# bottledspace/refraction-raytracing-dxr

Hardware: AMD Instinct MI355X
Metric: Mrays/s (primary+refracted) at 1920x1080, monkey.obj (higher is better)
Workload: dtype f32

## Files before the change

### refraction_raytracing_dxr_amd/csrc/rr_capi.cpp

```cpp
#include "../../include/rrdxr.h"

#include <hip/hip_runtime.h>

#include <algorithm>
#include <cmath>
#include <cstdio>
#include <cstdlib>
#include <cstring>
#include <new>
#include <string>
#include <vector>

#include "rr_launch.h"

using namespace rr;

static_assert(sizeof(rr_vertex) == 32, "Vertex stride (Mesh.cpp:45)");
static_assert(sizeof(rr_instance_desc) == 64, "D3D12_RAYTRACING_INSTANCE_DESC");
static_assert(sizeof(rr_scene_constants) == 80, "SceneConstants");
static_assert(sizeof(rr_ray) == sizeof(rr_ray_dev) && sizeof(rr_hit) == sizeof(rr_hit_dev), "ray/hit ABI");
static_assert(offsetof(rr_ray, instance_mask) == 36 && offsetof(rr_ray_dev, instance_mask) == 36, "rr_ray.instance_mask");

#include <dlfcn.h>
struct rr_nccl_unique_id { char internal[128]; };
// ... 127 lines not shown
    size_t    park_bytes[MAX_LANES + 1] = {};
    char       last_kernel_name[96] = "";
    uint32_t   last_kernel = 0;
    uint32_t* d_tickets = nullptr;

    int  dbg_kernel = 0;
    int  dbg_stack = 0;
    int  dbg_ticket_blocks = 0;
    bool dbg_group_trace = true;
    bool dbg_async_set = false;
    uint32_t dbg_async[2] = { 2, 2 };
    bool dbg_tile_order = true;
    int  dbg_stream_waves = 6;
    bool dbg_tlas32 = false;
    int  dbg_shape = 0;
    std::string dbg_diag;

    hipEvent_t ev_begin = nullptr, ev_end = nullptr;
    std::vector<hipEvent_t> kev;
    uint32_t kev_used = 0;

    StreamDev strm[MAX_LANES + 1] = {};
    size_t    strm_cap[MAX_LANES + 1] = {};
    size_t    strm_pixels[MAX_LANES + 1] = {};
    size_t    strm_budget = 0;
    struct KernelChoice {
        int choice = 0;
        uint32_t seen = 0;
        unsigned long long key = 0;
        double share = 0.0;
// ... 13 lines not shown
                if (x.stamp < lru->stamp) lru = &x;
            }
            *lru = KernelChoice();
            lru->valid = true; lru->key = key; lru->stamp = clock;
            return lru;
        }
        const KernelChoice* peek(unsigned long long key) const
        {
            for (const KernelChoice& x : e) if (x.valid && x.key == key) return &x;
            return nullptr;
        }
    };
    static unsigned long long choice_key(uint32_t width, uint32_t height, const rr_dispatch_params& p, uint32_t depth)
    {
        return ((unsigned long long)width << 48) ^ ((unsigned long long)height << 32) ^ ((unsigned long long)(uint32_t)p.max_refract << 8) ^
               ((unsigned long long)(uint32_t)p.max_reflect << 4) ^ (depth <= 2 ? depth : depth < 8 ? 3u : depth < 24 ? 4u : depth < 48 ? 5u : 6u);
    }
    ChoiceClass ch_tlas, ch_many, ch_few;
    hipEvent_t ch_ev[4] = {};

    rr_ray_dev* d_rays = nullptr;
    rr_hit_dev* d_hits = nullptr;
    uint32_t ray_cap = 0;
};

namespace {

int fail(rr_context* ctx, int code, const char* what, hipError_t e = hipSuccess)
{
    if (ctx) {
        ctx->err = what;
// ... 162 lines not shown
        hipMalloc(&ctx->d_cnt, sizeof(CounterBlock)) != hipSuccess ||
        hipMalloc(&ctx->d_tickets, (rr_context::MAX_LANES + 1) * LDS_TICKET_WORDS * sizeof(uint32_t)) != hipSuccess) {
        if (ctx->own_stream) (void)hipStreamDestroy(ctx->own_stream);
        dfree(ctx->d_cnt);
        delete ctx;
        return RR_ERR_DEVICE;
    }
    ctx->stream = ctx->own_stream;
    (void)hipMemsetAsync(ctx->d_cnt, 0, sizeof(CounterBlock), ctx->stream);
    (void)hipMemsetAsync(ctx->d_tickets, 0, (rr_context::MAX_LANES + 1) * LDS_TICKET_WORDS * sizeof(uint32_t), ctx->stream);
    if (const char* e = getenv("RR_DEBUG_KERNEL"))
        ctx->dbg_kernel = !strcmp(e, "fused") ? 1 : !strcmp(e, "lds") ? 4 : !strcmp(e, "paths") ? 5 : !strcmp(e, "stream") ? 10 : 0;
    if (const char* e = getenv("RR_DEBUG_STACK")) ctx->dbg_stack = atoi(e);
    if (const char* e = getenv("RR_DEBUG_TICKET")) ctx->dbg_ticket_blocks = atoi(e);
    if (const char* e = getenv("RR_DEBUG_SHAPE")) ctx->dbg_shape = atoi(e);
    if (const char* e = getenv("RR_DEBUG_TLAS32")) ctx->dbg_tlas32 = atoi(e) != 0;
    if (const char* e = getenv("RR_DEBUG_TILE_ORDER")) ctx->dbg_tile_order = atoi(e) != 0;
    if (const char* e = getenv("RR_DEBUG_ASYNC")) { unsigned l = 2, sh = 2; if (sscanf(e, "%u,%u", &l, &sh) == 2 && l >= 1 && sh >= 1) { ctx->dbg_async[0] = l; ctx->dbg_async[1] = sh; ctx->dbg_async_set = true; } }
    if (const char* e = getenv("RR_DEBUG_DIAG")) ctx->dbg_diag = e;
    if (const char* e = getenv("RR_DEBUG_GROUP_TRACE")) ctx->dbg_group_trace = atoi(e) != 0;
    *out = ctx;
    return RR_OK;
}

int rr_destroy(rr_context* ctx)
{
    if (!ctx) return RR_ERR_INVALID_ARGUMENT;
    (void)hipSetDevice(ctx->device);
    (void)hipStreamSynchronize(ctx->stream);
    for (uint32_t l = 0; l < rr_context::MAX_LANES; ++l) {
// ... 543 lines not shown
constexpr size_t STREAM_BUDGET_MAX = (size_t)48 << 30, STREAM_BUDGET_MIN = (size_t)1 << 30;
constexpr uint32_t STREAM_BLK = 1024;

size_t stream_budget(rr_context* ctx)
{
    if (ctx->strm_budget == 0) {
        size_t free_b = 0, total_b = 0;
        size_t b = STREAM_BUDGET_MAX;
        if (hipMemGetInfo(&free_b, &total_b) == hipSuccess) b = std::min(b, free_b / 6u);
        if (const char* e = getenv("RR_DEBUG_STREAM_BUDGET_GB")) { const long g = atol(e); if (g > 0 && g <= 200) b = (size_t)g << 30; }
        ctx->strm_budget = std::max(b, STREAM_BUDGET_MIN);
    }
    return ctx->strm_budget;
}

inline bool lds_default_depth(uint32_t depth) { return depth >= 24u; }

bool scene_fits_lds(const rr_context* ctx)
{
    if (!ctx->single_identity || ctx->dbg_stack != 0 || ctx->inst_host.empty()) return false;
    const MeshRes& m0 = ctx->meshes[(size_t)ctx->inst_host[0].blas];
    const uint32_t node_bytes = (m0.n_tris > 1 ? m0.n_tris - 1 : 1) * (uint32_t)sizeof(QNode);
    return m0.n_tris < 32768u && lds_kernel_shape(node_bytes, scene_stack_need(ctx) + 1, nullptr, ctx->dbg_shape) >= 0;
}

uint32_t stream_slot(const rr_context* ctx)
{
    for (uint32_t l = 0; l < rr_context::MAX_LANES; ++l) if (ctx->lane_stream[l] && ctx->stream == ctx->lane_stream[l]) return l;
    return rr_context::MAX_LANES;
}

struct StreamPlan { uint32_t fc, n_wg; size_t cap, pixels; };

size_t stream_rect_wb(const DispatchDev& a, uint32_t frames)
{
    const size_t all = (size_t)a.blocks_per_frame * frames * 4u;
    if (!a.mesh_part && a.rt_w == 0u) return all;
    const size_t tiles = a.mesh_part ? (size_t)a.n_mesh_local : (size_t)a.rt_w * a.rt_h;
// ... 178 lines not shown
        RR_HIP(hipMemsetAsync(d_diag, 0, diag_waves * 64, ctx->stream));
        a.diag = d_diag;
    }

    const bool stats = (p.flags & RR_DISPATCH_COLLECT_STATS) != 0;
    const uint32_t need = scene_stack_need(ctx);
    const bool keep = keep_counters || (p.flags & RR_DISPATCH_KEEP_COUNTERS) != 0;
    const uint32_t filled = mesh ? n_mesh_local : local;
    if (compact && filled < max_local)
        for (uint32_t f = 0; f < depth; ++f)
            RR_HIP(hipMemsetAsync(reinterpret_cast<uint8_t*>(a.out_rgba8 + f * stride) + (size_t)filled * TILE * TILE * (rgb8 ? 3 : 4), 0,
                                  (size_t)(max_local - filled) * TILE * TILE * (rgb8 ? 3 : 4), ctx->stream));
    int stack_sel = need <= 19 ? 19 : need <= 22 ? 22 : need <= 26 ? 26 : need <= 31 ? 31 : need <= 39 ? 39 : 64;
    if (ctx->dbg_stack >= (int)need) stack_sel = ctx->dbg_stack;
    const MeshRes* m0 = ctx->single_identity ? &ctx->meshes[(size_t)ctx->inst_host[0].blas] : nullptr;
    const uint32_t node_bytes = m0 ? (m0->n_tris > 1 ? m0->n_tris - 1 : 1) * (uint32_t)sizeof(QNode) : 0;
    const double rect_share = (double)(a.hx1 - a.hx0) * (double)(a.hy1 - a.hy0) / ((double)width * (double)height);
    const bool lds_fits = scene_fits_lds(ctx) && (uint64_t)a.n_tiles * depth * depth < 0x40000000ull;
    const bool have_rect = a.hx1 > a.hx0 && a.hy1 > a.hy0;
    uint32_t pool_nodes = 0;
    if (!ctx->single_identity) {
        pool_nodes = ctx->n_insts > 1 ? ctx->n_insts - 1 : 1;
        std::vector<char> seen(ctx->meshes.size(), 0);
        for (uint32_t i = 0; i < ctx->n_insts; ++i) {
            const size_t mi = (size_t)ctx->inst_host[i].blas;
            if (!seen[mi]) { seen[mi] = 1; pool_nodes += ctx->meshes[mi].n_tris > 1 ? ctx->meshes[mi].n_tris - 1 : 1; }
        }
    }
    const bool refill_stack16 = ctx->single_identity ? (m0 && m0->n_tris < 32768u && need > 19)
                                                     : (pool_nodes < 32768u && ctx->n_pool_tris + ctx->n_insts < 32768u);
    const bool stream_ok = !ctx->single_identity && p.max_reflect <= 2 && p.max_refract <= (int)STREAM_MAX_GEN - 2 && refill_stack16 && need <= 39 &&
// ... 25 lines not shown
    auto launch_lds = [&](bool st) -> int {
        LdsDispatch q;
        memset(&q, 0, sizeof q);
        const uint32_t slot = lds_slot();
        q.tickets = ctx->d_tickets + (size_t)slot * LDS_TICKET_WORDS;
        q.park_slots = p.max_reflect <= 2 ? 2u : 8u;
        if (int r = ensure_lds_park(slot)) return r;
        q.park = ctx->d_park[slot];
        uint32_t rect[4];
        mesh_screen_rect(m0->bounds, ((ctx->dbg_ticket_blocks & 3) == 1 || (p.flags & RR_DISPATCH_DEBUG_NO_CULL)) ? nullptr : h_cams, depth, width, height, rect);
        const int tk = ctx->dbg_ticket_blocks & 3;
        if (tk == 2) rect[2] = rect[0];
        q.n_queues = (ctx->dbg_ticket_blocks & 64) ? 64u : (ctx->dbg_ticket_blocks & 128) ? LDS_QUEUES : 8u;
        q.home_xcc = (ctx->dbg_ticket_blocks & 16) ? 0u : 1u;
        q.rx0 = rect[0]; q.ry0 = rect[1]; q.rx1 = rect[2]; q.ry1 = rect[3];
        q.node_bytes = node_bytes;
        q.stack_entries = need + 1;
        RR_HIP(launch_render_lds(sc, a, q, ctx->n_cus, st, ctx->stream, ctx->dbg_shape));
        return RR_OK;
    };
    auto launch_paths = [&](bool st) -> int { RR_HIP(launch_render_paths(sc, a, (int)need, st, ctx->stream)); return RR_OK; };
    auto launch_stream = [&](bool st) -> int { return render_stream(ctx, sc, a, depth, (int)need, st, rgb8); };

    enum { K_FUSED = 0, K_LDS = 1, K_PATHS = 2, K_STREAM = 7 };
    int kernel = K_FUSED;
    rr_context::ChoiceClass* cls = nullptr;
    int cand_a = K_FUSED, cand_b = K_FUSED;
    if (ctx->dbg_kernel == 10) { if (stream_ok) kernel = K_STREAM; }
    else if (ctx->dbg_kernel == 5) { if (paths_ok) kernel = K_PATHS; }
    else if (ctx->dbg_kernel == 4) { if (lds_fits && !mesh && !compact) kernel = K_LDS; }
    else if (ctx->dbg_kernel == 0 && !a.diag) {
        if (stream_ok) { cls = &ctx->ch_tlas; cand_b = K_STREAM; }
        else if (paths_ok) { cls = &ctx->ch_few; cand_b = K_PATHS; }
// ... 805 lines not shown
```

### refraction_raytracing_dxr_amd/csrc/rr_device.h

```cpp
#pragma once
#include <hip/hip_runtime.h>
#include "rr_types.h"

namespace rr {

struct f3 { float x, y, z; };

__device__ __forceinline__ f3 mk3(float x, float y, float z) { f3 r; r.x = x; r.y = y; r.z = z; return r; }
__device__ __forceinline__ f3 sub3(f3 a, f3 b) { return mk3(a.x - b.x, a.y - b.y, a.z - b.z); }
__device__ __forceinline__ f3 neg3(f3 a) { return mk3(-a.x, -a.y, -a.z); }
__device__ __forceinline__ f3 scale3(f3 a, float s) { return mk3(a.x * s, a.y * s, a.z * s); }
__device__ __forceinline__ float dot3(f3 a, f3 b) { return fmaf(a.z, b.z, fmaf(a.y, b.y, a.x * b.x)); }
__device__ __forceinline__ f3 cross3(f3 a, f3 b)
{
    return mk3(fmaf(a.y, b.z, -(a.z * b.y)), fmaf(a.z, b.x, -(a.x * b.z)), fmaf(a.x, b.y, -(a.y * b.x)));
}
__device__ __forceinline__ f3 normalize3(f3 a)
{
    float inv = 1.0f / sqrtf(dot3(a, a));
    return scale3(a, inv);
}

__device__ __forceinline__ float rr_atan2f(float y, float x)
{
// ... 85 lines not shown
    BoxRay r;
    box_axis(O.x, D.x, eps_w, g.org[0], g.cell[0], r.inv.x, r.kn.x, r.kf.x, r.sx);
    box_axis(O.y, D.y, eps_w, g.org[1], g.cell[1], r.inv.y, r.kn.y, r.kf.y, r.sy);
    box_axis(O.z, D.z, eps_w, g.org[2], g.cell[2], r.inv.z, r.kn.z, r.kf.z, r.sz);
    return r;
}

struct NodeQ { uint4 a, b; };
__device__ __forceinline__ NodeQ load_node(const QNode* __restrict__ nodes, int node)
{
    const uint4* q = reinterpret_cast<const uint4*>(reinterpret_cast<const char*>(nodes) + (uint32_t)node);
    NodeQ n;
    n.a = q[0]; n.b = q[1];
    return n;
}
struct GlobalNodes {
    __device__ __forceinline__ NodeQ load(const QNode* __restrict__ nodes, int node) const { return load_node(nodes, node); }
};
struct LdsNodes {
    const char* base;
    __device__ __forceinline__ NodeQ load(const QNode* __restrict__, int node) const
    {
        const uint4* q = reinterpret_cast<const uint4*>(base + (uint32_t)node);
        NodeQ n;
        n.a = q[0]; n.b = q[1];
        return n;
    }
};


constexpr int TRAV_DONE = (int)0x80000000;

typedef float v2f __attribute__((ext_vector_type(2)));
__device__ __forceinline__ v2f splat2(float x) { v2f r = { x, x }; return r; }
__device__ __forceinline__ v2f mk2(float x, float y) { v2f r = { x, y }; return r; }

__device__ __forceinline__ float vmax3(float a, float b, float c) { float r; asm("v_max3_f32 %0, %1, %2, %3" : "=v"(r) : "v"(a), "v"(b), "v"(c)); return r; }
__device__ __forceinline__ float vmin3(float a, float b, float c) { float r; asm("v_min3_f32 %0, %1, %2, %3" : "=v"(r) : "v"(a), "v"(b), "v"(c)); return r; }
__device__ __forceinline__ float vmax2(float a, float b) { float r; asm("v_max_f32 %0, %1, %2" : "=v"(r) : "v"(a), "v"(b)); return r; }
__device__ __forceinline__ float vmin2(float a, float b) { float r; asm("v_min_f32 %0, %1, %2" : "=v"(r) : "v"(a), "v"(b)); return r; }

typedef _Float16 h2v __attribute__((ext_vector_type(2)));
// ... 5 lines not shown
    const uint32_t lox = n.a.x, loy = n.a.y, loz = n.a.z, hix = n.a.w, hiy = n.b.x, hiz = n.b.y;
    const v2f nx = RR_PLANE2(r.sx ? hix : lox, r.inv.x, r.kn.x);
    const v2f ny = RR_PLANE2(r.sy ? hiy : loy, r.inv.y, r.kn.y);
    const v2f nz = RR_PLANE2(r.sz ? hiz : loz, r.inv.z, r.kn.z);
    const v2f fx = RR_PLANE2(r.sx ? lox : hix, r.inv.x, r.kf.x);
    const v2f fy = RR_PLANE2(r.sy ? loy : hiy, r.inv.y, r.kf.y);
    const v2f fz = RR_PLANE2(r.sz ? loz : hiz, r.inv.z, r.kf.z);
    tn0 = vmax2(vmax3(nx.x, ny.x, nz.x), tmin);
    tn1 = vmax2(vmax3(nx.y, ny.y, nz.y), tmin);
    const float tf0 = vmin2(vmin3(fx.x, fy.x, fz.x), tmax);
    const float tf1 = vmin2(vmin3(fx.y, fy.y, fz.y), tmax);
    h0 = tn0 <= tf0;
    h1 = tn1 <= tf1;
}

constexpr int STACK_STRIDE = 64;
template <class E> struct StackCodec;
template <> struct StackCodec<uint32_t> {
    static __device__ __forceinline__ uint32_t enc(int ref) { return (uint32_t)ref; }
    static __device__ __forceinline__ int dec(uint32_t v) { return (int)v; }
};
template <> struct StackCodec<uint16_t> {
    static __device__ __forceinline__ uint16_t enc(int ref) { const int n = ref >> 5; return (uint16_t)(n < ref ? n : ref); }
    static __device__ __forceinline__ int dec(uint16_t v) { const int s = (int)(int16_t)v, n = s << 5; return n > s ? n : s; }
};

template <class E>
__device__ __forceinline__ int node_step(const BoxRay& br, const NodeQ& n, float tmin, float tmax, E*& top, const E* floor)
{
    bool h0, h1;
    float tn0, tn1;
    box2_hit(br, n, tmin, tmax, h0, h1, tn0, tn1);
    const int c0 = (int)n.b.z, c1 = (int)n.b.w;
    const bool both = h0 && h1, swap = tn1 < tn0;
    const int nearc = (h0 && !(h1 && swap)) ? c0 : c1;
    int next = (h0 || h1) ? nearc : TRAV_DONE;
    if (both) { *top = StackCodec<E>::enc(swap ? c0 : c1); top += STACK_STRIDE; }
    if (!(h0 || h1) && top > floor) { top -= STACK_STRIDE; next = StackCodec<E>::dec(*top); }
    return next;
}

struct Diag { uint32_t* trips; uint32_t stride = 4; };
__device__ __forceinline__ void diag_trip(const Diag& d, int which = 0)
{
    if (d.trips) { const unsigned long long m = __ballot(1); if ((int)(threadIdx.x & 63u) == __ffsll((long long)m) - 1) d.trips[which * d.stride] += 1u; }
}


__device__ __forceinline__ void tri_test(const TriRec* __restrict__ tris, uint32_t leaf, f3 O, f3 D, float tmin,
                                         uint32_t cull, uint32_t inst, HitRec& best)
{
    const float4* q = reinterpret_cast<const float4*>(tris + leaf);
    float4 a = q[0], b = q[1], c = q[2];
    f3 v0 = mk3(a.x, a.y, a.z), e1 = mk3(b.x, b.y, b.z), e2 = mk3(c.x, c.y, c.z);
    uint32_t prim = __float_as_uint(a.w);
// ... 37 lines not shown
__device__ __forceinline__ bool leaf_phase_due(int n_in)
{
    const int quarter = n_in >> 2;
    const int thr = quarter > 2 ? quarter : 2;
    return __popcll(__ballot(1)) + thr <= n_in;
}

template <bool STATS, class E, class NS = GlobalNodes, bool ANY = false>
__device__ __forceinline__ void walk_blas(const QNode* __restrict__ nodes, const TriRec* __restrict__ tris, int root, const BoxRay& br,
                                          f3 O, f3 D, float tmin, uint32_t cull, uint32_t inst, HitRec& best, E* stk,
                                          TravCounters& cnt, const Diag dg = Diag{ nullptr }, const NS ns = NS{},
                                          bool any_lane = false)
{
    E* top = stk;
    int node = root;
    for (;;) {
        const int n_in = __popcll(__ballot(node >= 0));
        while (node >= 0) {
            if (leaf_phase_due(n_in)) break;
            diag_trip(dg);
            const NodeQ q = ns.load(nodes, node);
            if (STATS) { cnt.nodes++; if (first_active_lane()) cnt.node_trips++; }
            node = node_step(br, q, tmin, best.t, top, stk);
#ifdef RR_EXP_EXTRA_VALU
            { float dv = br.inv.x;
#pragma unroll
              for (int k = 0; k < RR_EXP_EXTRA_VALU; ++k) asm volatile("v_add_f32 %0, %0, %0" : "+v"(dv));
              asm volatile("" :: "v"(dv)); }
#endif
        }
        if (node < 0 && node != TRAV_DONE) {
            diag_trip(dg, 1);
            if (STATS) { cnt.tris++; if (first_active_lane()) cnt.leaf_trips++; }
            tri_test(tris, (uint32_t)~node, O, D, tmin, cull, inst, best);
            if (ANY && any_lane && best.hit) { top = stk; node = TRAV_DONE; }
            else if (top > stk) { top -= STACK_STRIDE; node = StackCodec<E>::dec(*top); } else node = TRAV_DONE;
        }
        if (__ballot(node != TRAV_DONE) == 0ull) break;
    }
}

template <bool STATS, class E, class NS = GlobalNodes>
__device__ __forceinline__ void trace_blas(const BlasDev& bl, f3 O, f3 D, float tmin, uint32_t cull, uint32_t inst,
                                           HitRec& best, E* stk, TravCounters& cnt, const Diag dg = Diag{ nullptr },
                                           const NS ns = NS{})
{
    const BoxRay br = box_ray(O, D, bl.scale, bl.grid);
    walk_blas<STATS, E, NS>(bl.nodes, bl.tris, 0, br, O, D, tmin, cull, inst, best, stk, cnt, dg, ns);
    if (best.hit) hit_attributes(bl.tris, O, D, best);
}

// ... 244 lines not shown
```

### refraction_raytracing_dxr_amd/csrc/rr_launch.h

```cpp
#pragma once
#include <hip/hip_runtime.h>
#include "rr_types.h"

namespace rr {

struct alignas(16) rr_ray_dev { float origin[3]; float tmin; float dir[3]; float tmax; uint32_t flags; uint32_t instance_mask; uint32_t pad[2]; };
struct rr_hit_dev { float t, u, v; uint32_t prim, inst, hit; };
static_assert(sizeof(rr_ray_dev) == 48 && sizeof(rr_hit_dev) == 24, "ABI layout");

hipError_t launch_render_fused(const SceneDev& sc, const DispatchDev& a, int stack, int pend, bool stats, hipStream_t s,
                               bool stack16 = false);
int lds_kernel_shape(uint32_t node_bytes, uint32_t stack_entries, size_t* lds_bytes, int min_shape = 0);
hipError_t launch_render_lds(const SceneDev& sc, const DispatchDev& a, LdsDispatch q, int n_cus, bool stats, hipStream_t s, int min_shape = 0);
hipError_t launch_render_paths(const SceneDev& sc, const DispatchDev& a, int stack, bool stats, hipStream_t s);
hipError_t launch_assemble_frames_mesh_rgb8(const uint8_t* gathered, const uint8_t* bg, uint32_t* frames, uint32_t W, uint32_t H, const MeshPartDev& mp,
                                            size_t rank_stride_b, size_t frame_stride_b, size_t bg_stride_b, size_t out_stride, uint32_t n_frames, hipStream_t s);
hipError_t launch_render_stream(const SceneDev& sc, const DispatchDev& a, const StreamDev& s, int stack, uint32_t n_wg, bool stats, hipStream_t st, int waves = 6);
const char* last_stream_kernel_name();
const char* last_render_kernel_name();
hipError_t launch_trace_rays(const SceneDev& sc, const rr_ray_dev* rays, uint32_t n, rr_hit_dev* hits, uint32_t* err,
                             int stack, hipStream_t s);
hipError_t launch_query_rays(const SceneDev& sc, const rr_ray_dev* rays, uint32_t n, rr_hit_dev* hits, uint32_t inst0_mask, int stack,
                             hipStream_t s);
hipError_t launch_screen_tables(float* out, uint32_t W, uint32_t H, hipStream_t s);
hipError_t launch_env_lookup(const SceneDev& sc, const float* dirs, uint32_t n, float* rgb, hipStream_t s);
hipError_t launch_assemble_tiles(const uint32_t* gathered, uint32_t* frame, uint32_t W, uint32_t H, uint32_t tiles_x,
                                 uint32_t n_tiles, uint32_t world, uint32_t max_tiles, hipStream_t s);
hipError_t launch_assemble_frames(const uint32_t* gathered, uint32_t* frames, uint32_t W, uint32_t H, uint32_t tiles_x,
// ... 42 lines not shown
```

### refraction_raytracing_dxr_amd/csrc/rr_render.hip

```cpp
#include <hip/hip_runtime.h>
#include <cstdlib>
#include <cstring>
#include "rr_render_common.h"

namespace rr {

template <int STACK, int PEND, bool STATS, bool TLAS, bool DIAG = false, class E = uint32_t, int WPS = 0>
__global__ __launch_bounds__(256, WPS ? WPS : TLAS ? RR_TLAS_WAVES_PER_SIMD(STACK) : sizeof(E) == 2 ? 8 : RR_FUSED_WAVES_PER_SIMD(STACK)) void k_render_fused(SceneDev sc, DispatchDev a)
{
    __shared__ uint32_t diag_trips[12];
    const unsigned long long diag_t0 = DIAG ? __builtin_amdgcn_s_memtime() : 0ull;
    const unsigned long long diag_rt0 = DIAG ? __builtin_amdgcn_s_memrealtime() : 0ull;
    if (DIAG && threadIdx.x < 12) diag_trips[threadIdx.x] = 0;
    if (DIAG) __syncthreads();
    extern __shared__ __attribute__((aligned(16))) uint32_t lds[];
    const uint32_t wave = __builtin_amdgcn_readfirstlane(threadIdx.x >> 6), lane = threadIdx.x & 63u;
    E* stk = reinterpret_cast<E*>(lds) + wave * (STACK * 64) + lane;

    const BlockPos bp = wave_block_pos(a, blockIdx.x * 4u + wave);
    const uint32_t lx = compact1by1(lane), ly = compact1by1(lane >> 1);
    const uint32_t x = bp.x0 + lx, y = bp.y0 + ly;
    const bool valid = bp.tile_ok && x < a.W && y < a.H;
    const CamDev& cb = a.cams[bp.frame];

// ... 208 lines not shown
    return p;
}

__device__ __forceinline__ BlockPos lds_rect_block(const DispatchDev& a, const LdsDispatch& q, uint32_t u, uint32_t j)
{
    BlockPos p;
    const uint32_t strip = a.n_frames == 1u ? u : __umulhi(u, q.div_frames), per_row = q.rect_bw >> 2;
    p.frame = u - strip * a.n_frames;
    const uint32_t row = per_row == 1u ? strip : __umulhi(strip, q.div_per_row), col = strip - row * per_row;
    p.tile_local = 0u; p.tile_ok = true; p.bg = false;
    p.px0 = 0u; p.py0 = 0u;
    p.x0 = q.rx0 + col * 32u + j * 8u; p.y0 = q.ry0 + row * 8u;
    return p;
}

template <int NW, int WGS, bool STATS, bool DIAG = false>
__global__ __launch_bounds__(NW * 64, NW * WGS / 4) void k_render_lds(SceneDev sc, DispatchDev a, LdsDispatch q)
{
    typedef uint16_t E;
    __shared__ uint32_t diag_tr[3 * 16];
    __shared__ uint32_t wg_arrived;
    __shared__ unsigned long long wg_share[16];
    if (threadIdx.x == 0) wg_arrived = 0u;
    if (threadIdx.x < 16) wg_share[threadIdx.x] = 0ull;
    const unsigned long long diag_t0 = DIAG ? __builtin_amdgcn_s_memtime() : 0ull;
    unsigned long long diag_wait = 0ull, diag_render = 0ull, diag_n = 0ull;
    unsigned long long diag_worst = 0ull, diag_worst_trips = 0ull;
    if (DIAG && threadIdx.x < 48) diag_tr[threadIdx.x] = 0;
    extern __shared__ __attribute__((aligned(16))) uint32_t lds[];
    {
        const uint4* __restrict__ src = reinterpret_cast<const uint4*>(sc.blas0.nodes);
        uint4* dst = reinterpret_cast<uint4*>(lds);
        for (uint32_t i = threadIdx.x; i < q.node_bytes / 16u; i += NW * 64) dst[i] = src[i];
    }
    __syncthreads();
    const unsigned long long diag_t1 = DIAG ? __builtin_amdgcn_s_memtime() : 0ull;
    const uint32_t wave = __builtin_amdgcn_readfirstlane(threadIdx.x >> 6), lane = threadIdx.x & 63u;
    const LdsNodes ns{ reinterpret_cast<const char*>(lds) };
    MemPark park{ q.park + (size_t)(blockIdx.x * NW + wave) * ((size_t)q.park_slots * 8 * 64) + lane };
    E* stk = reinterpret_cast<E*>(reinterpret_cast<char*>(lds) + q.node_bytes) + wave * (q.stack_entries * 64u) + lane;
    const uint32_t lx = compact1by1(lane), ly = compact1by1(lane >> 1);

    LaneStats st;
    stats_clock_begin<STATS>(st);
    auto in_rect = [&](const BlockPos& bp) { return bp.x0 >= q.rx0 && bp.x0 < q.rx1 && bp.y0 >= q.ry0 && bp.y0 < q.ry1; };
    const uint32_t NQ = q.n_queues;
    uint32_t home = (blockIdx.x * NW + wave) % NQ;
    if (q.home_xcc) { uint32_t xcc; asm volatile("s_getreg_b32 %0, hwreg(HW_REG_XCC_ID)" : "=s"(xcc)); home = (xcc & 7u) % NQ; }
    uint32_t phase = 0, qi = home, tried = 0;
    for (;;) {
        BlockPos bp;
        bool have = false;
        while (!have) {
// ... 49 lines not shown
                if (lane == 0) wg_share[wave] = ((unsigned long long)((u + 1u) | 0x80000000u) << 32) | 1ull;
                bp = lds_tile_block(a, q, u, 0u);
                have = bp.tile_ok && !in_rect(bp);
            }
        }
        if (!have) break;
        st.blocks += 1u;
        const unsigned long long dr0 = DIAG ? __builtin_amdgcn_s_memtime() : 0ull;
        const uint32_t dI0 = DIAG ? diag_tr[wave] : 0u, dL0 = DIAG ? diag_tr[16 + wave] : 0u, dS0 = DIAG ? diag_tr[32 + wave] : 0u;
        const uint32_t x = bp.x0 + lx, y = bp.y0 + ly;
        const bool may_hit = bp.x0 + 8u > a.hx0 && bp.x0 < a.hx1 && bp.y0 + 8u > a.hy0 && bp.y0 < a.hy1;
        if (STATS && !may_hit) st.bg_blocks += 1u;
        if (x < a.W && y < a.H) {
            const CamDev& cb = a.cams[bp.frame];
            st.pixels += 1;
            const f3 acc = render_pixel<STATS, false, DIAG, E, LdsNodes>(sc, a, cb, x, y, may_hit, stk, ns, park, st, Diag{ DIAG ? &diag_tr[wave] : nullptr, 16 });
            const size_t o = a.compact_out == 0u ? (size_t)y * a.W + x
                                                : (size_t)bp.tile_local * (TILE * TILE) + (bp.py0 + ly) * TILE + (bp.px0 + lx);
            store_pixel(a, a.out_rgba8 + (size_t)bp.frame * a.frame_stride,
                        a.out_f32 ? a.out_f32 + (size_t)bp.frame * a.frame_stride : nullptr, o, acc);
        }
        if (DIAG) {
            const unsigned long long dt = __builtin_amdgcn_s_memtime() - dr0;
            diag_render += dt; diag_n += 1ull << 32;
            if (dt > diag_worst) {
                diag_worst = dt;
                diag_worst_trips = (unsigned long long)(diag_tr[wave] - dI0) | ((unsigned long long)(diag_tr[16 + wave] - dL0) << 20) |
                                   ((unsigned long long)(diag_tr[32 + wave] - dS0) << 40);
            }
        }
    }
    if (DIAG && lane == 0) {
        unsigned long long* d = a.diag + (size_t)(blockIdx.x * NW + wave) * 8;
        d[0] = diag_wait; d[1] = diag_render; d[2] = diag_n; d[3] = __builtin_amdgcn_s_memtime() - diag_t0;
        d[4] = diag_worst; d[5] = diag_worst_trips; d[6] = diag_t1 - diag_t0; d[7] = diag_tr[wave] | ((unsigned long long)diag_tr[16 + wave] << 32);
    }
    flush_stats<STATS>(a, st, blockIdx.x * NW + wave, lane);
    if (lane == 0) {
        const uint32_t w_arrived = atomicAdd(&wg_arrived, 1u);
        if (w_arrived + 1u == (uint32_t)NW) {
            const uint32_t arrived = atomicAdd(&q.tickets[2u * LDS_QUEUES * 16u], 1u);
            if (arrived + 1u == gridDim.x) {
                for (uint32_t k = 0; k <= 2u * LDS_QUEUES; ++k) atomicExch(&q.tickets[k * 16u], 0u);
            }
        }
    }
}

__global__ __launch_bounds__(256) void k_screen_tables(float* out, uint32_t W, uint32_t H)
{
    const uint32_t i = blockIdx.x * 256u + threadIdx.x;
    if (i < W) out[i] = screen_coord(i, W, false);
    else if (i < W + H) out[i] = screen_coord(i - W, H, true);
}

__global__ __launch_bounds__(256) void k_env_lookup(SceneDev sc, const float* dirs, uint32_t n, float* rgb)
{
    const uint32_t i = blockIdx.x * 256u + threadIdx.x;
    if (i >= n) return;
    const f3 e = env_lookup(sc, mk3(dirs[i * 3], dirs[i * 3 + 1], dirs[i * 3 + 2]));
    rgb[i * 3] = e.x; rgb[i * 3 + 1] = e.y; rgb[i * 3 + 2] = e.z;
// ... 168 lines not shown
}

static thread_local char g_kernel_name[96] = "";
const char* last_render_kernel_name() { return g_kernel_name; }
#define RR_NAME(...) snprintf(g_kernel_name, sizeof g_kernel_name, __VA_ARGS__)
template <int STACK, int PEND, bool TLAS>
static hipError_t launch_fused_spt(const SceneDev& sc, const DispatchDev& a, bool stats, hipStream_t s)
{
    const size_t lds = (size_t)4 * STACK * 64 * sizeof(uint32_t);
    RR_NAME("k_render_fused<%d, %d, %s, %s, false, unsigned int, 0>", STACK, PEND, stats ? "true" : "false", TLAS ? "true" : "false");
    if (stats) hipLaunchKernelGGL((k_render_fused<STACK, PEND, true, TLAS>), dim3(a.n_blocks), dim3(256), lds, s, sc, a);
    else       hipLaunchKernelGGL((k_render_fused<STACK, PEND, false, TLAS>), dim3(a.n_blocks), dim3(256), lds, s, sc, a);
    return hipGetLastError();
}

template <int NW, int WGS>
static hipError_t launch_lds_nw(const SceneDev& sc, const DispatchDev& a, const LdsDispatch& q, size_t lds, int n_cus, bool stats, hipStream_t s)
{
    static const hipError_t attr = [] {
        hipError_t e = hipFuncSetAttribute(reinterpret_cast<const void*>(&k_render_lds<NW, WGS, false>), hipFuncAttributeMaxDynamicSharedMemorySize, 159 * 1024);
        if (e == hipSuccess) e = hipFuncSetAttribute(reinterpret_cast<const void*>(&k_render_lds<NW, WGS, true>), hipFuncAttributeMaxDynamicSharedMemorySize, 159 * 1024);
        return e;
    }();
    if (attr != hipSuccess) return attr;
    const dim3 grid((uint32_t)n_cus * WGS), block(NW * 64);
    RR_NAME("k_render_lds<%d, %d, %s, false>", NW, WGS, stats ? "true" : "false");
    if (stats) hipLaunchKernelGGL((k_render_lds<NW, WGS, true>), grid, block, lds, s, sc, a, q);
    else       hipLaunchKernelGGL((k_render_lds<NW, WGS, false>), grid, block, lds, s, sc, a, q);
    return hipGetLastError();
}

int lds_kernel_shape(uint32_t node_bytes, uint32_t stack_entries, size_t* lds_bytes, int min_shape)
{
    static const struct { int nw, wgs; } shapes[] = { { 12, 2 }, { 16, 2 }, { 16, 1 } };
    for (int i = min_shape < 0 ? 0 : min_shape; i < 3; ++i) {
        const size_t need = (size_t)node_bytes + (size_t)shapes[i].nw * stack_entries * 64 * sizeof(uint16_t);
        if (need <= (size_t)(160 * 1024) / shapes[i].wgs - 512) { if (lds_bytes) *lds_bytes = need; return i; }
        if (min_shape <= 0) break;
    }
    return -1;
}

hipError_t launch_render_lds(const SceneDev& sc, const DispatchDev& a, LdsDispatch q, int n_cus, bool stats, hipStream_t s, int min_shape)
{
    if (a.n_blocks == 0) return hipSuccess;
    size_t lds = 0;
    const int shape = lds_kernel_shape(q.node_bytes, q.stack_entries, &lds, min_shape);
    if (shape < 0) return hipErrorInvalidValue;
    {
        static const int wgs[] = { 2, 2, 1 };
        const uint32_t grid = (uint32_t)n_cus * (uint32_t)wgs[shape];
        if (q.n_queues > grid) q.n_queues = grid;
        if (q.n_queues > LDS_QUEUES) q.n_queues = LDS_QUEUES;
        if (q.n_queues < 1u) q.n_queues = 1u;
    }
    q.p2_tickets = a.n_local_tiles * a.n_frames;
    if (q.rx1 > q.rx0 && q.ry1 > q.ry0) {
        q.rx0 &= ~31u;
        q.rx1 = (q.rx1 + 31u) & ~31u;
    }
    const bool rect = q.rx1 > q.rx0 && q.ry1 > q.ry0;
    q.rect_bw = rect ? (q.rx1 - q.rx0) / 8u : 0u;
    q.p1_tickets = !rect ? 0u : (q.rect_bw / 4u) * ((q.ry1 - q.ry0) / 8u) * a.n_frames;
    if ((uint64_t)q.p2_tickets * a.n_frames >= 0xffffffffull || (uint64_t)q.p1_tickets * a.n_frames >= 0xffffffffull) return hipErrorInvalidValue;
    q.div_frames = (uint32_t)(0x100000000ull / a.n_frames) + 1u;
    q.div_tiles_x = (uint32_t)(0x100000000ull / a.tiles_x) + 1u;
    q.div_per_row = rect ? (uint32_t)(0x100000000ull / (q.rect_bw / 4u)) + 1u : 0u;
    if (a.diag) {
        static const hipError_t attr = hipFuncSetAttribute(reinterpret_cast<const void*>(&k_render_lds<12, 2, false, true>), hipFuncAttributeMaxDynamicSharedMemorySize, 159 * 1024);
        if (attr != hipSuccess) return attr;
        const size_t l12 = (size_t)q.node_bytes + (size_t)12 * q.stack_entries * 64 * sizeof(uint16_t);
        hipLaunchKernelGGL((k_render_lds<12, 2, false, true>), dim3((uint32_t)n_cus * 2), dim3(12 * 64), l12, s, sc, a, q);
        return hipGetLastError();
    }
    if (shape == 0) return launch_lds_nw<12, 2>(sc, a, q, lds, n_cus, stats, s);
    if (shape == 1) return launch_lds_nw<16, 2>(sc, a, q, lds, n_cus, stats, s);
    return launch_lds_nw<16, 1>(sc, a, q, lds, n_cus, stats, s);
}

template <int STACK, int PEND>
static hipError_t launch_fused_sp(const SceneDev& sc, const DispatchDev& a, bool stats, hipStream_t s)
{
    if (!sc.single_identity) return launch_fused_spt<STACK, PEND, true>(sc, a, stats, s);
    return launch_fused_spt<STACK, PEND, false>(sc, a, stats, s);
}

template <int PEND>
static hipError_t launch_fused_s16(const SceneDev& sc, const DispatchDev& a, bool stats, hipStream_t s)
{
    const size_t lds = (size_t)4 * 39 * 64 * sizeof(uint16_t);
    RR_NAME("k_render_fused<39, %d, %s, false, false, unsigned short, 0>", PEND, stats ? "true" : "false");
    if (stats) hipLaunchKernelGGL((k_render_fused<39, PEND, true, false, false, uint16_t>), dim3(a.n_blocks), dim3(256), lds, s, sc, a);
// ... 139 lines not shown
```

Before: 31210.

## Add sign-indexed 44-byte LDS node layout for BVH traversal

Introduces an alternative LDS node format in which each BVH node is expanded into per-axis plane pairs ordered by ray direction sign, with child references pre-scaled to byte offsets. Traversal then loads only the near/far planes each ray needs, using a simpler plane-slab test and a matching stack codec. The old 32-byte quantized layout remains available through an env switch, and the depth threshold for picking the LDS kernel is lowered from 24 to 20. The cost is larger node storage in LDS, which may force a different workgroup shape or fall back when the node count is too high, plus extra template instantiations.

```diff
diff --git a/refraction_raytracing_dxr_amd/csrc/rr_capi.cpp b/refraction_raytracing_dxr_amd/csrc/rr_capi.cpp
--- a/refraction_raytracing_dxr_amd/csrc/rr_capi.cpp
+++ b/refraction_raytracing_dxr_amd/csrc/rr_capi.cpp
@@ -165,6 +165,7 @@
     int  dbg_stream_waves = 6;
     bool dbg_tlas32 = false;
     int  dbg_shape = 0;
+    bool dbg_lds32 = false;
     std::string dbg_diag;
 
     hipEvent_t ev_begin = nullptr, ev_end = nullptr;
@@ -208,7 +209,7 @@
     static unsigned long long choice_key(uint32_t width, uint32_t height, const rr_dispatch_params& p, uint32_t depth)
     {
         return ((unsigned long long)width << 48) ^ ((unsigned long long)height << 32) ^ ((unsigned long long)(uint32_t)p.max_refract << 8) ^
-               ((unsigned long long)(uint32_t)p.max_reflect << 4) ^ (depth <= 2 ? depth : depth < 8 ? 3u : depth < 24 ? 4u : depth < 48 ? 5u : 6u);
+               ((unsigned long long)(uint32_t)p.max_reflect << 4) ^ (depth <= 2 ? depth : depth < 8 ? 3u : depth < 20 ? 4u : depth < 48 ? 5u : 6u);
     }
     ChoiceClass ch_tlas, ch_many, ch_few;
     hipEvent_t ch_ev[4] = {};
@@ -401,6 +402,7 @@
     if (const char* e = getenv("RR_DEBUG_STACK")) ctx->dbg_stack = atoi(e);
     if (const char* e = getenv("RR_DEBUG_TICKET")) ctx->dbg_ticket_blocks = atoi(e);
     if (const char* e = getenv("RR_DEBUG_SHAPE")) ctx->dbg_shape = atoi(e);
+    if (const char* e = getenv("RR_DEBUG_LDS_LAYOUT")) ctx->dbg_lds32 = atoi(e) == 32;
     if (const char* e = getenv("RR_DEBUG_TLAS32")) ctx->dbg_tlas32 = atoi(e) != 0;
     if (const char* e = getenv("RR_DEBUG_TILE_ORDER")) ctx->dbg_tile_order = atoi(e) != 0;
     if (const char* e = getenv("RR_DEBUG_ASYNC")) { unsigned l = 2, sh = 2; if (sscanf(e, "%u,%u", &l, &sh) == 2 && l >= 1 && sh >= 1) { ctx->dbg_async[0] = l; ctx->dbg_async[1] = sh; ctx->dbg_async_set = true; } }
@@ -974,14 +976,14 @@
     return ctx->strm_budget;
 }
 
-inline bool lds_default_depth(uint32_t depth) { return depth >= 24u; }
+inline bool lds_default_depth(uint32_t depth) { return depth >= 20u; }
 
 bool scene_fits_lds(const rr_context* ctx)
 {
     if (!ctx->single_identity || ctx->dbg_stack != 0 || ctx->inst_host.empty()) return false;
     const MeshRes& m0 = ctx->meshes[(size_t)ctx->inst_host[0].blas];
-    const uint32_t node_bytes = (m0.n_tris > 1 ? m0.n_tris - 1 : 1) * (uint32_t)sizeof(QNode);
-    return m0.n_tris < 32768u && lds_kernel_shape(node_bytes, scene_stack_need(ctx) + 1, nullptr, ctx->dbg_shape) >= 0;
+    const uint32_t n_nodes = m0.n_tris > 1 ? m0.n_tris - 1 : 1;
+    return m0.n_tris < 32768u && lds_kernel_shape(n_nodes, scene_stack_need(ctx) + 1, nullptr, ctx->dbg_shape, !ctx->dbg_lds32) >= 0;
 }
 
 uint32_t stream_slot(const rr_context* ctx)
@@ -1190,7 +1192,7 @@
     int stack_sel = need <= 19 ? 19 : need <= 22 ? 22 : need <= 26 ? 26 : need <= 31 ? 31 : need <= 39 ? 39 : 64;
     if (ctx->dbg_stack >= (int)need) stack_sel = ctx->dbg_stack;
     const MeshRes* m0 = ctx->single_identity ? &ctx->meshes[(size_t)ctx->inst_host[0].blas] : nullptr;
-    const uint32_t node_bytes = m0 ? (m0->n_tris > 1 ? m0->n_tris - 1 : 1) * (uint32_t)sizeof(QNode) : 0;
+    const uint32_t n_nodes = m0 ? (m0->n_tris > 1 ? m0->n_tris - 1 : 1) : 0;
     const double rect_share = (double)(a.hx1 - a.hx0) * (double)(a.hy1 - a.hy0) / ((double)width * (double)height);
     const bool lds_fits = scene_fits_lds(ctx) && (uint64_t)a.n_tiles * depth * depth < 0x40000000ull;
     const bool have_rect = a.hx1 > a.hx0 && a.hy1 > a.hy0;
@@ -1246,9 +1248,8 @@
         q.n_queues = (ctx->dbg_ticket_blocks & 64) ? 64u : (ctx->dbg_ticket_blocks & 128) ? LDS_QUEUES : 8u;
         q.home_xcc = (ctx->dbg_ticket_blocks & 16) ? 0u : 1u;
         q.rx0 = rect[0]; q.ry0 = rect[1]; q.rx1 = rect[2]; q.ry1 = rect[3];
-        q.node_bytes = node_bytes;
         q.stack_entries = need + 1;
-        RR_HIP(launch_render_lds(sc, a, q, ctx->n_cus, st, ctx->stream, ctx->dbg_shape));
+        RR_HIP(launch_render_lds(sc, a, q, n_nodes, ctx->n_cus, st, ctx->stream, ctx->dbg_shape, !ctx->dbg_lds32));
         return RR_OK;
     };
     auto launch_paths = [&](bool st) -> int { RR_HIP(launch_render_paths(sc, a, (int)need, st, ctx->stream)); return RR_OK; };
diff --git a/refraction_raytracing_dxr_amd/csrc/rr_device.h b/refraction_raytracing_dxr_amd/csrc/rr_device.h
--- a/refraction_raytracing_dxr_amd/csrc/rr_device.h
+++ b/refraction_raytracing_dxr_amd/csrc/rr_device.h
@@ -123,8 +123,11 @@
     n.a = q[0]; n.b = q[1];
     return n;
 }
+struct NoNodeRay {};
 struct GlobalNodes {
     __device__ __forceinline__ NodeQ load(const QNode* __restrict__ nodes, int node) const { return load_node(nodes, node); }
+    __device__ __forceinline__ NoNodeRay ray(const BoxRay&) const { return NoNodeRay{}; }
+    __device__ __forceinline__ NodeQ load(const QNode* __restrict__ nodes, int node, NoNodeRay) const { return load(nodes, node); }
 };
 struct LdsNodes {
     const char* base;
@@ -135,6 +138,8 @@
         n.a = q[0]; n.b = q[1];
         return n;
     }
+    __device__ __forceinline__ NoNodeRay ray(const BoxRay&) const { return NoNodeRay{}; }
+    __device__ __forceinline__ NodeQ load(const QNode* __restrict__ nodes, int node, NoNodeRay) const { return load(nodes, node); }
 };
 
 
@@ -170,6 +175,22 @@
     h1 = tn1 <= tf1;
 }
 
+__device__ __forceinline__ void box2_planes(const BoxRay& r, uint32_t nxw, uint32_t nyw, uint32_t nzw, uint32_t fxw, uint32_t fyw,
+                                            uint32_t fzw, float tmin, float tmax, bool& h0, bool& h1, float& tn0, float& tn1)
+{
+    const v2f nx = RR_PLANE2(nxw, r.inv.x, r.kn.x);
+    const v2f ny = RR_PLANE2(nyw, r.inv.y, r.kn.y);
+    const v2f nz = RR_PLANE2(nzw, r.inv.z, r.kn.z);
+    const v2f fx = RR_PLANE2(fxw, r.inv.x, r.kf.x);
+    const v2f fy = RR_PLANE2(fyw, r.inv.y, r.kf.y);
+    const v2f fz = RR_PLANE2(fzw, r.inv.z, r.kf.z);
+    tn0 = vmax2(vmax3(nx.x, ny.x, nz.x), tmin);
+    tn1 = vmax2(vmax3(nx.y, ny.y, nz.y), tmin);
+    const float tf0 = vmin2(vmin3(fx.x, fy.x, fz.x), tmax);
+    const float tf1 = vmin2(vmin3(fx.y, fy.y, fz.y), tmax);
+    h0 = tn0 <= tf0;
+    h1 = tn1 <= tf1;
+}
 constexpr int STACK_STRIDE = 64;
 template <class E> struct StackCodec;
 template <> struct StackCodec<uint32_t> {
@@ -181,20 +202,65 @@
     static __device__ __forceinline__ int dec(uint16_t v) { const int s = (int)(int16_t)v, n = s << 5; return n > s ? n : s; }
 };
 
+template <class C, class E>
+__device__ __forceinline__ int node_next(bool h0, bool h1, float tn0, float tn1, int c0, int c1, E*& top, const E* floor)
+{
+    const bool both = h0 && h1, swap = tn1 < tn0;
+    const int nearc = (h0 && !(h1 && swap)) ? c0 : c1;
+    int next = (h0 || h1) ? nearc : TRAV_DONE;
+    if (both) { *top = C::enc(swap ? c0 : c1); top += STACK_STRIDE; }
+    if (!(h0 || h1) && top > floor) { top -= STACK_STRIDE; next = C::dec(*top); }
+    return next;
+}
 template <class E>
 __device__ __forceinline__ int node_step(const BoxRay& br, const NodeQ& n, float tmin, float tmax, E*& top, const E* floor)
 {
     bool h0, h1;
     float tn0, tn1;
     box2_hit(br, n, tmin, tmax, h0, h1, tn0, tn1);
-    const int c0 = (int)n.b.z, c1 = (int)n.b.w;
-    const bool both = h0 && h1, swap = tn1 < tn0;
-    const int nearc = (h0 && !(h1 && swap)) ? c0 : c1;
-    int next = (h0 || h1) ? nearc : TRAV_DONE;
-    if (both) { *top = StackCodec<E>::enc(swap ? c0 : c1); top += STACK_STRIDE; }
-    if (!(h0 || h1) && top > floor) { top -= STACK_STRIDE; next = StackCodec<E>::dec(*top); }
-    return next;
-}
+    return node_next<StackCodec<E>>(h0, h1, tn0, tn1, (int)n.b.z, (int)n.b.w, top, floor);
+}
+
+constexpr uint32_t LDS_SIGN_NODE_BYTES = 44;
+struct StackCodecSign {
+    static __device__ __forceinline__ uint16_t enc(int ref) { const int n = ref >> 2; return (uint16_t)(n < ref ? n : ref); }
+    static __device__ __forceinline__ int dec(uint16_t v) { const int s = (int)(int16_t)v, n = s << 2; return n > s ? n : s; }
+};
+struct NodeSign { uint32_t nx, ny, nz, fx, fy, fz; int c0, c1; };
+struct SignNodeRay { uint32_t ox, oy, oz; };
+struct LdsSignNodes {
+    const char* base;
+    __device__ __forceinline__ SignNodeRay ray(const BoxRay& br) const
+    {
+        SignNodeRay k;
+        k.ox = br.sx ? 0u : 4u; k.oy = br.sy ? 0u : 4u; k.oz = br.sz ? 0u : 4u;
+        return k;
+    }
+    __device__ __forceinline__ NodeSign load(const QNode* __restrict__, int node, const SignNodeRay& k) const
+    {
+        const char* p = base + (uint32_t)node;
+        const uint32_t* x = reinterpret_cast<const uint32_t*>(p + k.ox);
+        const uint32_t* y = reinterpret_cast<const uint32_t*>(p + k.oy) + 3;
+        const uint32_t* z = reinterpret_cast<const uint32_t*>(p + k.oz) + 6;
+        const int32_t* c = reinterpret_cast<const int32_t*>(p) + 9;
+        NodeSign n;
+        n.nx = x[0]; n.fx = x[1];
+        n.ny = y[0]; n.fy = y[1];
+        n.nz = z[0]; n.fz = z[1];
+        n.c0 = c[0]; n.c1 = c[1];
+        return n;
+    }
+};
+template <class E>
+__device__ __forceinline__ int node_step(const BoxRay& br, const NodeSign& n, float tmin, float tmax, E*& top, const E* floor)
+{
+    bool h0, h1;
+    float tn0, tn1;
+    box2_planes(br, n.nx, n.ny, n.nz, n.fx, n.fy, n.fz, tmin, tmax, h0, h1, tn0, tn1);
+    return node_next<StackCodecSign>(h0, h1, tn0, tn1, n.c0, n.c1, top, floor);
+}
+template <class NS, class E> struct NodeCodec { typedef StackCodec<E> T; };
+template <> struct NodeCodec<LdsSignNodes, uint16_t> { typedef StackCodecSign T; };
 
 struct Diag { uint32_t* trips; uint32_t stride = 4; };
 __device__ __forceinline__ void diag_trip(const Diag& d, int which = 0)
@@ -262,12 +328,13 @@
 {
     E* top = stk;
     int node = root;
+    const auto nk = ns.ray(br);
     for (;;) {
         const int n_in = __popcll(__ballot(node >= 0));
         while (node >= 0) {
             if (leaf_phase_due(n_in)) break;
             diag_trip(dg);
-            const NodeQ q = ns.load(nodes, node);
+            const auto q = ns.load(nodes, node, nk);
             if (STATS) { cnt.nodes++; if (first_active_lane()) cnt.node_trips++; }
             node = node_step(br, q, tmin, best.t, top, stk);
 #ifdef RR_EXP_EXTRA_VALU
@@ -282,7 +349,7 @@
             if (STATS) { cnt.tris++; if (first_active_lane()) cnt.leaf_trips++; }
             tri_test(tris, (uint32_t)~node, O, D, tmin, cull, inst, best);
             if (ANY && any_lane && best.hit) { top = stk; node = TRAV_DONE; }
-            else if (top > stk) { top -= STACK_STRIDE; node = StackCodec<E>::dec(*top); } else node = TRAV_DONE;
+            else if (top > stk) { top -= STACK_STRIDE; node = NodeCodec<NS, E>::T::dec(*top); } else node = TRAV_DONE;
         }
         if (__ballot(node != TRAV_DONE) == 0ull) break;
     }
diff --git a/refraction_raytracing_dxr_amd/csrc/rr_launch.h b/refraction_raytracing_dxr_amd/csrc/rr_launch.h
--- a/refraction_raytracing_dxr_amd/csrc/rr_launch.h
+++ b/refraction_raytracing_dxr_amd/csrc/rr_launch.h
@@ -10,8 +10,10 @@
 
 hipError_t launch_render_fused(const SceneDev& sc, const DispatchDev& a, int stack, int pend, bool stats, hipStream_t s,
                                bool stack16 = false);
-int lds_kernel_shape(uint32_t node_bytes, uint32_t stack_entries, size_t* lds_bytes, int min_shape = 0);
-hipError_t launch_render_lds(const SceneDev& sc, const DispatchDev& a, LdsDispatch q, int n_cus, bool stats, hipStream_t s, int min_shape = 0);
+struct LdsShape { int shape; bool sign; uint32_t node_bytes; size_t lds_bytes; };
+int lds_kernel_shape(uint32_t n_nodes, uint32_t stack_entries, LdsShape* out, int min_shape = 0, bool allow_sign = true);
+hipError_t launch_render_lds(const SceneDev& sc, const DispatchDev& a, LdsDispatch q, uint32_t n_nodes, int n_cus, bool stats, hipStream_t s,
+                             int min_shape = 0, bool allow_sign = true);
 hipError_t launch_render_paths(const SceneDev& sc, const DispatchDev& a, int stack, bool stats, hipStream_t s);
 hipError_t launch_assemble_frames_mesh_rgb8(const uint8_t* gathered, const uint8_t* bg, uint32_t* frames, uint32_t W, uint32_t H, const MeshPartDev& mp,
                                             size_t rank_stride_b, size_t frame_stride_b, size_t bg_stride_b, size_t out_stride, uint32_t n_frames, hipStream_t s);
diff --git a/refraction_raytracing_dxr_amd/csrc/rr_render.hip b/refraction_raytracing_dxr_amd/csrc/rr_render.hip
--- a/refraction_raytracing_dxr_amd/csrc/rr_render.hip
+++ b/refraction_raytracing_dxr_amd/csrc/rr_render.hip
@@ -1,6 +1,7 @@
 #include <hip/hip_runtime.h>
 #include <cstdlib>
 #include <cstring>
+#include <type_traits>
 #include "rr_render_common.h"
 
 namespace rr {
@@ -246,8 +247,8 @@
     return p;
 }
 
-template <int NW, int WGS, bool STATS, bool DIAG = false>
-__global__ __launch_bounds__(NW * 64, NW * WGS / 4) void k_render_lds(SceneDev sc, DispatchDev a, LdsDispatch q)
+template <int NW, int WGS, bool STATS, bool DIAG, class NS>
+__device__ __forceinline__ void render_lds(const SceneDev& sc, const DispatchDev& a, const LdsDispatch& q)
 {
     typedef uint16_t E;
     __shared__ uint32_t diag_tr[3 * 16];
@@ -260,7 +261,19 @@
     unsigned long long diag_worst = 0ull, diag_worst_trips = 0ull;
     if (DIAG && threadIdx.x < 48) diag_tr[threadIdx.x] = 0;
     extern __shared__ __attribute__((aligned(16))) uint32_t lds[];
-    {
+    if constexpr (std::is_same<NS, LdsSignNodes>::value) {
+        const uint4* __restrict__ src = reinterpret_cast<const uint4*>(sc.blas0.nodes);
+        const uint32_t n = q.node_bytes / LDS_SIGN_NODE_BYTES;
+        for (uint32_t i = threadIdx.x; i < n; i += NW * 64) {
+            const uint4 na = src[2 * i], nb = src[2 * i + 1];
+            uint32_t* d = lds + i * (LDS_SIGN_NODE_BYTES / 4u);
+            d[0] = na.w; d[1] = na.x; d[2] = na.w;
+            d[3] = nb.x; d[4] = na.y; d[5] = nb.x;
+            d[6] = nb.y; d[7] = na.z; d[8] = nb.y;
+            d[9]  = (int)nb.z >= 0 ? (nb.z >> 5) * LDS_SIGN_NODE_BYTES : nb.z;
+            d[10] = (int)nb.w >= 0 ? (nb.w >> 5) * LDS_SIGN_NODE_BYTES : nb.w;
+        }
+    } else {
         const uint4* __restrict__ src = reinterpret_cast<const uint4*>(sc.blas0.nodes);
         uint4* dst = reinterpret_cast<uint4*>(lds);
         for (uint32_t i = threadIdx.x; i < q.node_bytes / 16u; i += NW * 64) dst[i] = src[i];
@@ -268,7 +281,7 @@
     __syncthreads();
     const unsigned long long diag_t1 = DIAG ? __builtin_amdgcn_s_memtime() : 0ull;
     const uint32_t wave = __builtin_amdgcn_readfirstlane(threadIdx.x >> 6), lane = threadIdx.x & 63u;
-    const LdsNodes ns{ reinterpret_cast<const char*>(lds) };
+    const NS ns{ reinterpret_cast<const char*>(lds) };
     MemPark park{ q.park + (size_t)(blockIdx.x * NW + wave) * ((size_t)q.park_slots * 8 * 64) + lane };
     E* stk = reinterpret_cast<E*>(reinterpret_cast<char*>(lds) + q.node_bytes) + wave * (q.stack_entries * 64u) + lane;
     const uint32_t lx = compact1by1(lane), ly = compact1by1(lane >> 1);
@@ -348,7 +361,7 @@
         if (x < a.W && y < a.H) {
             const CamDev& cb = a.cams[bp.frame];
             st.pixels += 1;
-            const f3 acc = render_pixel<STATS, false, DIAG, E, LdsNodes>(sc, a, cb, x, y, may_hit, stk, ns, park, st, Diag{ DIAG ? &diag_tr[wave] : nullptr, 16 });
+            const f3 acc = render_pixel<STATS, false, DIAG, E, NS>(sc, a, cb, x, y, may_hit, stk, ns, park, st, Diag{ DIAG ? &diag_tr[wave] : nullptr, 16 });
             const size_t o = a.compact_out == 0u ? (size_t)y * a.W + x
                                                 : (size_t)bp.tile_local * (TILE * TILE) + (bp.py0 + ly) * TILE + (bp.px0 + lx);
             store_pixel(a, a.out_rgba8 + (size_t)bp.frame * a.frame_stride,
@@ -379,6 +392,16 @@
             }
         }
     }
+}
+template <int NW, int WGS, bool STATS, bool DIAG = false>
+__global__ __launch_bounds__(NW * 64, NW * WGS / 4) void k_render_lds(SceneDev sc, DispatchDev a, LdsDispatch q)
+{
+    render_lds<NW, WGS, STATS, DIAG, LdsSignNodes>(sc, a, q);
+}
+template <int NW, int WGS, bool STATS, bool DIAG = false>
+__global__ __launch_bounds__(NW * 64, NW * WGS / 4) void k_render_lds_q32(SceneDev sc, DispatchDev a, LdsDispatch q)
+{
+    render_lds<NW, WGS, STATS, DIAG, LdsNodes>(sc, a, q);
 }
 
 __global__ __launch_bounds__(256) void k_screen_tables(float* out, uint32_t W, uint32_t H)
@@ -577,39 +600,52 @@
     return hipGetLastError();
 }
 
-template <int NW, int WGS>
+template <int NW, int WGS, bool SIGN>
 static hipError_t launch_lds_nw(const SceneDev& sc, const DispatchDev& a, const LdsDispatch& q, size_t lds, int n_cus, bool stats, hipStream_t s)
 {
-    static const hipError_t attr = [] {
-        hipError_t e = hipFuncSetAttribute(reinterpret_cast<const void*>(&k_render_lds<NW, WGS, false>), hipFuncAttributeMaxDynamicSharedMemorySize, 159 * 1024);
-        if (e == hipSuccess) e = hipFuncSetAttribute(reinterpret_cast<const void*>(&k_render_lds<NW, WGS, true>), hipFuncAttributeMaxDynamicSharedMemorySize, 159 * 1024);
+    auto kern = [](bool st) {
+        if (SIGN) return st ? &k_render_lds<NW, WGS, true> : &k_render_lds<NW, WGS, false>;
+        return st ? &k_render_lds_q32<NW, WGS, true> : &k_render_lds_q32<NW, WGS, false>;
+    };
+    static const hipError_t attr = [&] {
+        hipError_t e = hipFuncSetAttribute(reinterpret_cast<const void*>(kern(false)), hipFuncAttributeMaxDynamicSharedMemorySize, 159 * 1024);
+        if (e == hipSuccess) e = hipFuncSetAttribute(reinterpret_cast<const void*>(kern(true)), hipFuncAttributeMaxDynamicSharedMemorySize, 159 * 1024);
         return e;
     }();
     if (attr != hipSuccess) return attr;
     const dim3 grid((uint32_t)n_cus * WGS), block(NW * 64);
-    RR_NAME("k_render_lds<%d, %d, %s, false>", NW, WGS, stats ? "true" : "false");
-    if (stats) hipLaunchKernelGGL((k_render_lds<NW, WGS, true>), grid, block, lds, s, sc, a, q);
-    else       hipLaunchKernelGGL((k_render_lds<NW, WGS, false>), grid, block, lds, s, sc, a, q);
-    return hipGetLastError();
-}
-
-int lds_kernel_shape(uint32_t node_bytes, uint32_t stack_entries, size_t* lds_bytes, int min_shape)
+    RR_NAME("%s<%d, %d, %s, false>", SIGN ? "k_render_lds" : "k_render_lds_q32", NW, WGS, stats ? "true" : "false");
+    hipLaunchKernelGGL(kern(stats), grid, block, lds, s, sc, a, q);
+    return hipGetLastError();
+}
+
+int lds_kernel_shape(uint32_t n_nodes, uint32_t stack_entries, LdsShape* out, int min_shape, bool allow_sign)
 {
     static const struct { int nw, wgs; } shapes[] = { { 12, 2 }, { 16, 2 }, { 16, 1 } };
     for (int i = min_shape < 0 ? 0 : min_shape; i < 3; ++i) {
-        const size_t need = (size_t)node_bytes + (size_t)shapes[i].nw * stack_entries * 64 * sizeof(uint16_t);
-        if (need <= (size_t)(160 * 1024) / shapes[i].wgs - 512) { if (lds_bytes) *lds_bytes = need; return i; }
+        for (int sign = allow_sign ? 1 : 0; sign >= 0; --sign) {
+            if (sign && (uint64_t)n_nodes * (LDS_SIGN_NODE_BYTES / 4u) >= 32768u) continue;
+            const uint32_t node_bytes = sign ? (n_nodes * LDS_SIGN_NODE_BYTES + 15u) & ~15u : n_nodes * (uint32_t)sizeof(QNode);
+            const size_t need = (size_t)node_bytes + (size_t)shapes[i].nw * stack_entries * 64 * sizeof(uint16_t);
+            if (need <= (size_t)(160 * 1024) / shapes[i].wgs - 512) {
+                if (out) { out->shape = i; out->sign = sign != 0; out->node_bytes = node_bytes; out->lds_bytes = need; }
+                return i;
+            }
+        }
         if (min_shape <= 0) break;
     }
     return -1;
 }
 
-hipError_t launch_render_lds(const SceneDev& sc, const DispatchDev& a, LdsDispatch q, int n_cus, bool stats, hipStream_t s, int min_shape)
+hipError_t launch_render_lds(const SceneDev& sc, const DispatchDev& a, LdsDispatch q, uint32_t n_nodes, int n_cus, bool stats, hipStream_t s,
+                             int min_shape, bool allow_sign)
 {
     if (a.n_blocks == 0) return hipSuccess;
-    size_t lds = 0;
-    const int shape = lds_kernel_shape(q.node_bytes, q.stack_entries, &lds, min_shape);
+    LdsShape ls;
+    const int shape = lds_kernel_shape(n_nodes, q.stack_entries, &ls, min_shape, allow_sign);
     if (shape < 0) return hipErrorInvalidValue;
+    const size_t lds = ls.lds_bytes;
+    q.node_bytes = ls.node_bytes;
     {
         static const int wgs[] = { 2, 2, 1 };
         const uint32_t grid = (uint32_t)n_cus * (uint32_t)wgs[shape];
@@ -630,15 +666,25 @@
     q.div_tiles_x = (uint32_t)(0x100000000ull / a.tiles_x) + 1u;
     q.div_per_row = rect ? (uint32_t)(0x100000000ull / (q.rect_bw / 4u)) + 1u : 0u;
     if (a.diag) {
-        static const hipError_t attr = hipFuncSetAttribute(reinterpret_cast<const void*>(&k_render_lds<12, 2, false, true>), hipFuncAttributeMaxDynamicSharedMemorySize, 159 * 1024);
+        auto kern = ls.sign ? &k_render_lds<12, 2, false, true> : &k_render_lds_q32<12, 2, false, true>;
+        static const hipError_t attr = [] {
+            hipError_t e = hipFuncSetAttribute(reinterpret_cast<const void*>(&k_render_lds<12, 2, false, true>), hipFuncAttributeMaxDynamicSharedMemorySize, 159 * 1024);
+            if (e == hipSuccess) e = hipFuncSetAttribute(reinterpret_cast<const void*>(&k_render_lds_q32<12, 2, false, true>), hipFuncAttributeMaxDynamicSharedMemorySize, 159 * 1024);
+            return e;
+        }();
         if (attr != hipSuccess) return attr;
         const size_t l12 = (size_t)q.node_bytes + (size_t)12 * q.stack_entries * 64 * sizeof(uint16_t);
-        hipLaunchKernelGGL((k_render_lds<12, 2, false, true>), dim3((uint32_t)n_cus * 2), dim3(12 * 64), l12, s, sc, a, q);
+        hipLaunchKernelGGL(kern, dim3((uint32_t)n_cus * 2), dim3(12 * 64), l12, s, sc, a, q);
         return hipGetLastError();
     }
-    if (shape == 0) return launch_lds_nw<12, 2>(sc, a, q, lds, n_cus, stats, s);
-    if (shape == 1) return launch_lds_nw<16, 2>(sc, a, q, lds, n_cus, stats, s);
-    return launch_lds_nw<16, 1>(sc, a, q, lds, n_cus, stats, s);
+    if (ls.sign) {
+        if (shape == 0) return launch_lds_nw<12, 2, true>(sc, a, q, lds, n_cus, stats, s);
+        if (shape == 1) return launch_lds_nw<16, 2, true>(sc, a, q, lds, n_cus, stats, s);
+        return launch_lds_nw<16, 1, true>(sc, a, q, lds, n_cus, stats, s);
+    }
+    if (shape == 0) return launch_lds_nw<12, 2, false>(sc, a, q, lds, n_cus, stats, s);
+    if (shape == 1) return launch_lds_nw<16, 2, false>(sc, a, q, lds, n_cus, stats, s);
+    return launch_lds_nw<16, 1, false>(sc, a, q, lds, n_cus, stats, s);
 }
 
 template <int STACK, int PEND>
```

After: 32090, median of 6. +2.8%, better.
